# michel-aractingi/soloRL

Hardware: AMD Instinct MI355X
Metric: env-steps/s (whole node) Solo12 walk, 4096 envs/GPU (higher is better)
Workload: dtype f32

## Files before the change

solorl_amd/csrc/solorl_hip.hip:

```cpp
#include <hip/hip_runtime.h>

#include <cmath>
#include <cstddef>
#include <cstdio>
#include <cstdlib>
#include <cstring>
#include <utility>
#include <string>
#include <vector>

#include "../../include/solorl.h"
#include "dynamics.hpp"
#include "perturb.hpp"

using namespace solo;

#ifndef SOLO_TU_PART
#define SOLO_TU_PART -1
#endif
extern "C" __attribute__((visibility("hidden"))) int solorl_fail_(int code, const char* msg);

namespace {

#if SOLO_TU_PART == -1 || SOLO_TU_PART == 4
// ... 444 lines not shown
SD void pol_fma(PolBatch<KB>& B, int K4, int k0, unsigned xoff, unsigned xoff_a, float (&c)[4], float (&a)[4]) {
  asm volatile("" ::: "memory");
#pragma unroll
  for (int kk = 0; kk < KB; kk++) { POL_PIN4(B.c[kk]); POL_PIN4(B.a[kk]); }
#pragma unroll
  for (int kk = 0; kk < KB; kk++)
    if (k0 + kk < K4) {
#pragma unroll
      for (int e = 0; e < 4; e++) {
        const nfloat4 xc = reinterpret_cast<const nfloat4*>(solo_smem + e * POL_ENV_BYTES + xoff)[k0 + kk];
        const nfloat4 xa = xoff_a == xoff ? xc : reinterpret_cast<const nfloat4*>(solo_smem + e * POL_ENV_BYTES + xoff_a)[k0 + kk];
        c[e] = pol_dot4(B.c[kk], xc, c[e]); a[e] = pol_dot4(B.a[kk], xa, a[e]);
      }
    }
}
SD void pol_act_store(const float (&c)[4], const float (&a)[4], unsigned yoff, int lane) {
#pragma unroll
  for (int e = 0; e < 4; e++) {
    float* y = reinterpret_cast<float*>(solo_smem + e * POL_ENV_BYTES + yoff);
    y[lane] = pol_tanh(c[e]); y[64 + lane] = pol_tanh(a[e]);
  }
}

template <int A>
SD void policy_tail_team(const PolicyTail& P, int O, int col, int t, idx_t env, bool valid) {
  float* const buf = reinterpret_cast<float*>(solo_smem + (unsigned)col * POL_ENV_BYTES);
  float* const h2 = buf + 224;
  const int lane = threadIdx.x & 63, O4 = O >> 2;
  static_assert(A < 15, "the critic head sits on lane 15");
  const bool head = t < A || t == 15;
  constexpr unsigned H1 = 96u * 4u, H2 = 224u * 4u;
  float c[4], a[4];
  PolBatch<11> w1a, w1b;
  PolBatch<8> w2a, w2b;
  nfloat4 whb[16];
  pol_load(w1a, P.cw0, P.aw0, O4, 0, lane);
  pol_load(w1b, P.cw0, P.aw0, O4, 11, lane);
#pragma unroll
  for (int e = 0; e < 4; e++) { c[e] = P.cb0[lane]; a[e] = P.ab0[lane]; }
  pol_fma(w1a, O4, 0, 0u, 0u, c, a);
  pol_load(w2a, P.cw1, P.aw1, 16, 0, lane);
  pol_fma(w1b, O4, 11, 0u, 0u, c, a);
  pol_act_store(c, a, H1, lane);
  pol_load(w2b, P.cw1, P.aw1, 16, 8, lane);
#pragma unroll
  for (int e = 0; e < 4; e++) { c[e] = P.cb1[lane]; a[e] = P.ab1[lane]; }
  TEAM_SYNC();
  pol_fma(w2a, 16, 0, H1, H1 + 256u, c, a);
  {
    gfloat4* wh = (gfloat4*)(t == 15 ? P.cw2 : P.mw + (size_t)(head ? t : 0) * 64);
#pragma unroll
    for (int k = 0; k < 16; k++) whb[k] = wh[k];
    asm volatile("" ::: "memory");
  }
  pol_fma(w2b, 16, 8, H1, H1 + 256u, c, a);
  pol_act_store(c, a, H2, lane);
  TEAM_SYNC();
  float out = 0.f;
  {
    asm volatile("" ::: "memory");
#pragma unroll
    for (int k = 0; k < 16; k++) POL_PIN4(whb[k]);
    const nfloat4* x = reinterpret_cast<const nfloat4*>(t == 15 ? h2 : h2 + 64);
    float o0 = t == 15 ? P.cb2[0] : P.mb[head ? t : 0], o1 = 0.f;
#pragma unroll
    for (int k = 0; k < 16; k += 2) { o0 = pol_dot4(whb[k], x[k], o0); o1 = pol_dot4(whb[k + 1], x[k + 1], o1); }
    out = head ? o0 + o1 : 0.f;
  }
  float lp = 0.f, act = out;
  if (t < A) {
    const float ls = P.logstd[t];
    const float nz = P.noise ? P.noise[(size_t)env * A + t] : 0.f;
    act = out + __expf(ls) * nz;
    lp = -0.5f * nz * nz - ls - POL_HALF_LOG_2PI;
  }
  lp = team_sum16(lp);
  if (valid) {
    if (t < A) P.action[(size_t)env * A + t] = act;
    if (t == 15) P.value[env] = out;
    if (t == 0) P.logp[env] = lp;
  }
}

template <typename T, int ROBOT, bool DUO = false>
SD void step_team(T* __restrict__ sf, int* __restrict__ si, const T* __restrict__ snf, const int* __restrict__ sni, int M,
                  const Layout& L, int N, const EnvParams& P, const PhysParams<T>& pp, const float* __restrict__ actions,
                  const Outputs& out, int mode) {
  using RB = Robot<ROBOT>;
  constexpr int NQ = RB::NQ, NPS = 13 + 2 * NQ;
  using LDS = RowLds<T, 4>;
  using CH = typename TeamCtx<T, ROBOT, LDS>::type;
  static_assert(sizeof(PhysState<T, NQ>) == NPS * sizeof(T), "PhysState is the HBM field order pos, quat, v, w, q, qd");
#ifdef SOLO_WAVE_TIMING
  long long wts_[11];
  for (int i_ = 0; i_ < 11; i_++) wts_[i_] = 0;
  const long long wr0_ = wall_clock64();
  if (threadIdx.x < 16) solo::solo_pt_acc[threadIdx.x] = 0;
  __syncthreads();
  wts_[0] = clock64();
#endif
  const unsigned wlane = DUO ? (threadIdx.x & 63u) : threadIdx.x;
  const int t = wlane & 15, col = wlane >> 4;
  const unsigned blk = (blockIdx.x & 7u) * (gridDim.x >> 3) + (blockIdx.x >> 3);
  idx_t e = (idx_t)blk * 4 + col;
  const bool valid = e < (idx_t)N;
  if (!valid) e = (idx_t)N - 1;
  const bool lead = valid && t == 0;
  LDS lds; lds.lanes = 4; lds.lane = col;
  if (P.lds_poison_on) {
    using TC = TeamCtx<T, ROBOT, LDS>;
    unsigned* w = reinterpret_cast<unsigned*>(solo_smem);
    for (unsigned k = wlane; k < TC::bytes / 4; k += 64) w[k] = P.lds_poison;
    __syncthreads();
  }
  const CH ch{col};
  SubCtx<T, ROBOT>& C = ch.get();
  T* const psv = reinterpret_cast<T*>(&C.ps);
  if constexpr (DUO) {
    if (blk * 4u >= (unsigned)N) return;
    if (__builtin_amdgcn_readfirstlane(threadIdx.x >> 6)) {
#pragma unroll 1
      for (int ss = 0; ss < P.frame_skip; ss++)
        substep_team_helper<T, ROBOT>(pp, lds, t, lead, valid, ss + 1 < P.frame_skip);
      duo_join_rows<T, ROBOT>();
      return;
    }
    if (!valid && t == 0) { C.mask = 0; C.nc = 0; C.nlim_total = 0; C.lsel = 0; C.smask = 0; }
  }
  idx_t env = 0;
  T a_t = T(0);
  if (valid) {
    env = P.linear_ids ? e : (idx_t)si[SX(I_ENVID, e, NI)];
    for (int f = t; f < NPS; f += 16) psv[f] = sf[SX(L.pos + f, e, L.NF)];
    if (t < NER) C.erec[t] = sf[SX(L.goal + t, e, L.NF)];
    if (t < 3) C.irec[t] = si[SX(t, e, NI)];
    for (int p = t; p < NPRIM; p += 16) C.lamp[p] = sf[SX(L.lam + p, e, L.NF)];
    if (t < NQ && mode == MODE_STEP) a_t = (T)actions[env * NQ + t];
  }
  static_assert(I_TIMESTEP == IR_TIMESTEP && I_MASK == IR_MASK && I_RNG == IR_RNG, "counter order");
  TEAM_SYNC();
  WT_STAMP(1);
  if (valid && t < NQ) {
    const T c = a_t < T(-1) ? T(-1) : (a_t > T(1) ? T(1) : a_t);
    T tq;
    if (P.control == SOLORL_CONTROL_TORQUE) tq = c * T(P.max_torque);
    else tq = clampv(T(P.kp) * (c * pp.qlim - C.ps.q[t]) - T(P.kd) * C.ps.qd[t], T(P.max_torque));
    C.tau_base[t] = mode == MODE_STEP ? tq : T(0);
    if (out.tau && mode == MODE_STEP) out.tau[env * NQ + t] = (float)tq;
  }
  const T asq = team_sum16(a_t * a_t);
  WT_STAMP(2);
  constexpr int HK = (DMAX + 15) / 16;
  T hk0[HK], hk1[HK];
#pragma unroll
  for (int k = 0; k < HK; k++) { hk0[k] = T(0); hk1[k] = T(0); }
  T csk[HK];
  if (L.H > 0) team_current_state<T, ROBOT, HK>(C, P.task, L.D, t, csk);
  TEAM_SYNC();
  if (lead) {
    C.erec[ER_XYPREV] = C.ps.pos.x; C.erec[ER_XYPREV + 1] = C.ps.pos.y;
    C.tmy = C.erec[ER_TMY];
    if constexpr (DUO) C.R0 = quat_to_mat(C.ps.qx, C.ps.qy, C.ps.qz, C.ps.qw);
  }
  if (valid && L.H > 0) {
#pragma unroll
    for (int k = 0; k < HK; k++) {
      const int d = t + 16 * k;
      if (d < L.D) {
        const T c = csk[k];
        for (int lv = L.H - 1; lv >= 2; lv--)
          sf[SX(L.hist + lv * HSTRIDE + d, e, L.NF)] = sf[SX(L.hist + (lv - 1) * HSTRIDE + d, e, L.NF)];
        if (L.H >= 2) { hk1[k] = sf[SX(L.hist + d, e, L.NF)]; sf[SX(L.hist + HSTRIDE + d, e, L.NF)] = hk1[k]; }
        sf[SX(L.hist + d, e, L.NF)] = c;
        hk0[k] = c;
      } else if (d < ((L.D + 3) & ~3)) {
        sf[SX(L.hist + d, e, L.NF)] = T(0);
        for (int lv = 1; lv < L.H; lv++) sf[SX(L.hist + lv * HSTRIDE + d, e, L.NF)] = T(0);
      }
    }
  }
  WT_STAMP(3);
#pragma unroll 1
  for (int ss = 0; ss < P.frame_skip; ss++) {
    const T sc = (ss == 0 || P.hold_torque) ? T(1) : T(0);
    if (valid && t < NQ) C.tau[t] = C.tau_base[t] * sc;
    const int m = substep_team<T, ROBOT, LDS, DUO>(pp, sf + SX(L.lam, e, L.NF), 4u, lds, t, lead, valid);
    if (lead) C.irec[IR_MASK] = m;
  }
  if constexpr (DUO) {
    duo_join_rows<T, ROBOT>();
  }
  WT_STAMP(4);
// ... 102 lines not shown
    if (with_policy) {
      TEAM_SYNC();
      policy_tail_team<NQ>(out.pol, L.D * (1 + L.H), col, t, env, valid);
    }
  }
  WT_STAMP(9);
#ifdef SOLO_WAVE_TIMING
  __builtin_amdgcn_s_waitcnt(0);
  if (threadIdx.x == 0 && blockIdx.x < solo::SOLO_WT_WAVES) {
    wts_[10] = clock64();
    unsigned long long* w_ = solo::solo_wave_times[blockIdx.x];
    w_[0] = (unsigned long long)(wts_[3] - wts_[0]); w_[1] = (unsigned long long)(wts_[4] - wts_[3]); w_[2] = (unsigned long long)(wts_[10] - wts_[4]);
    w_[3] = (unsigned long long)(wall_clock64() - wr0_);
    for (int i_ = 0; i_ < 10; i_++) w_[6 + i_] = (unsigned long long)(wts_[i_ + 1] > wts_[i_] && wts_[i_] ? wts_[i_ + 1] - wts_[i_] : 0);
    for (int i_ = 0; i_ < 10; i_++) w_[16 + i_] = solo::solo_pt_acc[i_];
    for (int i_ = 10; i_ < 14; i_++) w_[18 + i_] = solo::solo_pt_acc[i_];
  }
#endif
}

template <typename T, int ROBOT>
__global__ void __launch_bounds__(64)
step_kernel(T* __restrict__ sf, int* __restrict__ si, const T* __restrict__ snf, const int* __restrict__ sni, int M,
            Layout L, int N, EnvParams P, PhysParams<T> pp, const float* __restrict__ actions, Outputs out, int mode) {
  step_body<T, ROBOT>(sf, si, snf, sni, M, L, N, P, pp, actions, out, mode);
}

#ifndef SOLO_WAVES_PER_SIMD
#define SOLO_WAVES_PER_SIMD 2
#endif
template <typename T, int ROBOT>
__global__ void __launch_bounds__(64, sizeof(T) == 8 ? 1 : SOLO_WAVES_PER_SIMD)
step_kernel_team(T* __restrict__ sf, int* __restrict__ si, const T* __restrict__ snf, const int* __restrict__ sni, int M,
                 Layout L, int N, EnvParams P, PhysParams<T> pp, const float* __restrict__ actions, Outputs out, int mode) {
  step_team<T, ROBOT>(sf, si, snf, sni, M, L, N, P, pp, actions, out, mode);
}

template <typename T, int ROBOT>
__global__ void __launch_bounds__(128, SOLO_WAVES_PER_SIMD)
duo_kernel_team(T* __restrict__ sf, int* __restrict__ si, const T* __restrict__ snf, const int* __restrict__ sni, int M,
                Layout L, int N, EnvParams P, PhysParams<T> pp, const float* __restrict__ actions, Outputs out, int mode) {
  static_assert(sizeof(T) == 4, "the helper wavefront is an fp32 kernel");
  step_team<T, ROBOT, true>(sf, si, snf, sni, M, L, N, P, pp, actions, out, mode);
}

template <typename T> struct RolloutArgs {
  T* sf; int* si; const T* snf; const int* sni; int M;
  Layout L; int N; EnvParams P; PhysParams<T> pp;
  const float* actions; Outputs out;
  int mode;
  int K, pol_last;
};
template <typename T> SD T* row_adv(T* p, size_t n) { return p ? p + n : p; }
template <typename T, int ROBOT>
__global__ void __launch_bounds__(64, sizeof(T) == 8 ? 1 : SOLO_WAVES_PER_SIMD)
rollout_kernel_team(const RolloutArgs<T> args) {
  using RA = RolloutArgs<T>;
  typedef const __attribute__((address_space(4))) char* kptr;
  constexpr size_t A = Robot<ROBOT>::NQ;
  const int K = args.K;
#pragma unroll 1
  for (int k = 0; k < K; k++) {
    kptr ap = (kptr)__builtin_amdgcn_kernarg_segment_ptr();
    asm volatile("" : "+s"(ap));
    const RA& a = *(const RA*)ap;
    const size_t r = (size_t)k * (size_t)a.N, O = (size_t)(a.L.D * (1 + a.L.H));
    Outputs o = a.out;
    o.obs += r * O; o.rew += r; o.done += r;
    o.timeout = row_adv(o.timeout, r); o.success = row_adv(o.success, r); o.nan_reset = row_adv(o.nan_reset, r);
    o.ep_len = row_adv(o.ep_len, r); o.ep_rew = row_adv(o.ep_rew, r); o.goals = row_adv(o.goals, r);
    o.dr0 = row_adv(o.dr0, r); o.dr1 = row_adv(o.dr1, r); o.dr2 = row_adv(o.dr2, r); o.dr3 = row_adv(o.dr3, r); o.dr4 = row_adv(o.dr4, r);
    o.tau = row_adv(o.tau, r * A);
    if (o.pol.value) {
      if (k + 1 < K || a.pol_last) {
        const size_t r1 = r + (size_t)a.N;
        o.pol.value += r1; o.pol.logp += r1; o.pol.action += r1 * A; o.pol.noise = row_adv(o.pol.noise, r1 * A);
      } else o.pol.value = nullptr;
    }
    step_team<T, ROBOT>(a.sf, a.si, a.snf, a.sni, a.M, a.L, a.N, a.P, a.pp, a.actions + r * A, o, a.mode);
    TEAM_SYNC();
  }
}

template <typename T, int ROBOT, bool MASKED>
__global__ void reset_kernel(T* sf, int* si, const T* snf, const int* sni, int M, Layout L, int N, EnvParams P, float* obs,
                             const unsigned char* mask) {
  const idx_t e = (idx_t)blockIdx.x * blockDim.x + threadIdx.x;
  if (e >= (idx_t)N) return;
  if constexpr (MASKED) { if (!mask[si[SX(I_ENVID, e, NI)]]) return; }
  Env<T, Robot<ROBOT>::NQ> E;
  load_env(E, sf, si, L, (idx_t)N, e);
  const idx_t env = (idx_t)si[SX(I_ENVID, e, NI)];
  reset_from_snapshot<T, ROBOT>(E, sf, L, (idx_t)N, e, env, snf, sni, M, P);
  if (obs) write_obs<T, ROBOT>(E, sf, L, (idx_t)N, e, env, P.task, obs);
  store_env(E, sf, si, L, (idx_t)N, e);
  si[SX(I_NEEDRESET, e, NI)] = 0;
}

template <typename T, int ROBOT>
__global__ void obs_kernel(const T* sf, const int* si, Layout L, int N, int task, float* obs) {
  const idx_t e = (idx_t)blockIdx.x * blockDim.x + threadIdx.x;
  if (e >= (idx_t)N) return;
  Env<T, Robot<ROBOT>::NQ> E;
  load_env(E, sf, si, L, (idx_t)N, e);
  write_obs<T, ROBOT>(E, sf, L, (idx_t)N, e, (idx_t)si[SX(I_ENVID, e, NI)], task, obs);
}

template <typename T>
__global__ void init_pose_kernel(T* sf, int* si, Layout L, int N, T tmy) {
  const idx_t e = (idx_t)blockIdx.x * blockDim.x + threadIdx.x;
  if (e >= (idx_t)N) return;
  for (int f = 0; f < L.NF; f++) sf[SX(f, e, L.NF)] = T(0);
  sf[SX(L.pos + 2, e, L.NF)] = T(0.35);
  sf[SX(L.quat + 3, e, L.NF)] = T(1);
  sf[SX(L.tmy, e, L.NF)] = tmy;
  for (int k = 0; k < NI; k++) si[SX(k, e, NI)] = 0;
  si[SX(I_NEEDRESET, e, NI)] = 1;
  si[SX(I_ENVID, e, NI)] = (int)e;
}

template <typename T>
__global__ void copy_env_kernel(const T* sf, const int* si, int N, int src, T* df, int* di, int M, int dst, int NF) {
  const int f = blockIdx.x * blockDim.x + threadIdx.x;
  if (f < NF) df[SX(f, (idx_t)dst, NF)] = sf[SX(f, (idx_t)src, NF)];
  if (f < NI) di[SX(f, (idx_t)dst, NI)] = si[SX(f, (idx_t)src, NI)];
}

__global__ void __launch_bounds__(256) sort_perm_kernel(const int* __restrict__ si, int N, int* __restrict__ perm) {
  __shared__ int cnt[256][9];
  __shared__ int base[9];
  const int t = threadIdx.x, nt = blockDim.x;
  const int chunk = (N + nt - 1) / nt, lo = t * chunk, hi = lo + chunk < N ? lo + chunk : N;
  int c[9] = {0, 0, 0, 0, 0, 0, 0, 0, 0};
  for (int i = lo; i < hi; i++) { int k = __popc(si[SX(I_MASK, (idx_t)i, NI)] & 0xFFFFFF); k = k > 8 ? 8 : k; c[k]++; }
#pragma unroll
  for (int k = 0; k < 9; k++) cnt[t][k] = c[k];
  __syncthreads();
  if (t < 9) {
    int run = 0;
    for (int j = 0; j < nt; j++) { int v = cnt[j][t]; cnt[j][t] = run; run += v; }
    base[t] = run;
  }
  __syncthreads();
  if (t == 0) { int run = 0; for (int k = 0; k < 9; k++) { int v = base[k]; base[k] = run; run += v; } }
  __syncthreads();
  int off[9];
#pragma unroll
  for (int k = 0; k < 9; k++) off[k] = base[k] + cnt[t][k];
  for (int i = lo; i < hi; i++) {
    int k = __popc(si[SX(I_MASK, (idx_t)i, NI)] & 0xFFFFFF); k = k > 8 ? 8 : k;
    int d = 0;
#pragma unroll
    for (int q = 0; q < 9; q++) if (q == k) d = off[q]++;
    perm[d] = i;
  }
}

template <typename T>
__global__ void gather_state_kernel(const T* __restrict__ sf, const int* __restrict__ si, const int* __restrict__ perm, int N,
                                    int NF, T* __restrict__ df, int* __restrict__ di) {
  const int j = blockIdx.x * blockDim.x + threadIdx.x;
  if (j >= N) return;
  const int src = perm[j];
  const int f = blockIdx.y;
  if (f < NF) df[SX(f, (idx_t)j, NF)] = sf[SX(f, (idx_t)src, NF)];
  else di[SX(f - NF, (idx_t)j, NI)] = si[SX(f - NF, (idx_t)src, NI)];
// ... 155 lines not shown
                const float* __restrict__ vpred, const float* __restrict__ ret, int m, int A, float clip, float value_coef,
                int clipped_value, float* __restrict__ g_mean, float* __restrict__ g_values, float* __restrict__ part) {
  extern __shared__ float red[];
  const int i = blockIdx.x * blockDim.x + threadIdx.x;
  const bool on = i < m;
  const float inv_m = 1.0f / (float)m;
  float vl = 0.f, al = 0.f, glp = 0.f;
  float lp = 0.f;
  if (on) {
    for (int j = 0; j < A; j++) {
      const float ls = logstd[j];
      const float z = (action[(size_t)i * A + j] - mean[(size_t)i * A + j]) * __expf(-ls);
      lp += -0.5f * z * z - ls - 0.91893853320467274178f;
    }
    const float ratio = __expf(lp - old_logp[i]);
    const float a = adv[i];
    const float s1 = ratio * a;
    const float rc = fminf(fmaxf(ratio, 1.0f - clip), 1.0f + clip);
    const float s2 = rc * a;
    al = -fminf(s1, s2);
    const float inside = (ratio >= 1.0f - clip && ratio <= 1.0f + clip) ? 1.0f : 0.0f;
    const float w = s1 < s2 ? 1.0f : (s1 > s2 ? inside : 0.5f * (1.0f + inside));
    glp = -a * ratio * w * inv_m;
    const float v = values[i], r = ret[i];
    const float u = v - r;
    float gv;
    if (clipped_value) {
      const float dvp = v - vpred[i];
      const float vc = vpred[i] + fminf(fmaxf(dvp, -clip), clip);
      const float wv = vc - r;
      const float ins = (dvp >= -clip && dvp <= clip) ? 1.0f : 0.0f;
      const float uu = u * u, ww = wv * wv;
      vl = 0.5f * fmaxf(uu, ww);
      gv = uu > ww ? u : (uu < ww ? wv * ins : 0.5f * (u + wv * ins));
    } else { vl = 0.5f * u * u; gv = u; }
    g_values[i] = value_coef * gv * inv_m;
  }
  auto block_sum = [&](float x) -> float {
    red[threadIdx.x] = x;
    __syncthreads();
    for (int s = 128; s > 0; s >>= 1) { if ((int)threadIdx.x < s) red[threadIdx.x] += red[threadIdx.x + s]; __syncthreads(); }
    const float r = red[0];
    __syncthreads();
    return r;
  };
  float* P = part + (size_t)blockIdx.x * (3 + A);
  const float svl = block_sum(vl), sal = block_sum(al);
  if (threadIdx.x == 0) { P[0] = svl; P[1] = sal; P[2] = (float)(min(m - (int)(blockIdx.x * blockDim.x), (int)blockDim.x)); }
  for (int j = 0; j < A; j++) {
    float gls = 0.f;
    if (on) {
      const float e = __expf(-logstd[j]);
      const float z = (action[(size_t)i * A + j] - mean[(size_t)i * A + j]) * e;
      g_mean[(size_t)i * A + j] = glp * z * e;
      gls = glp * (z * z - 1.0f);
    }
    const float s = block_sum(gls);
    if (threadIdx.x == 0) P[3 + j] = s;
  }
}

}

struct solorl_env {
  solorl_config cfg;
  int N = 0, device = 0, n = 0, D = 0, O = 0, M = 0;
  bool f64 = false, reset_called = false;
  size_t tsize = 4;
  Layout L;
  void* sf = nullptr; int* si = nullptr; void* snf = nullptr; int* sni = nullptr;
  void* sf2 = nullptr; int* si2 = nullptr; int* perm = nullptr;
  bool sort = true;
  uint64_t seed = 0; int64_t id0 = 0;
  double goal_radius = 2.0;
  double* dyn = nullptr;
  std::vector<unsigned> stab_host;
  unsigned* stab = nullptr;
  bool spread = true;
  bool team = false;
  int lds_poison_on = 0; unsigned lds_poison = 0;
  int simds = 1024;
  int pipe_override = -1;
  int helper_override = -1;
  int* pert_countdown = nullptr; unsigned* pert_kicks = nullptr;
  PerturbParams pert{};
};

namespace {

EnvParams make_env_params(const solorl_env* h) {
  EnvParams P;
  const solorl_config& c = h->cfg;
  P.task = c.task; P.control = c.control; P.frame_skip = c.frame_skip; P.episode_length = c.episode_length;
  P.hold_torque = c.hold_torque; P.disable_termination = c.disable_termination;
  P.settle_min = c.settle_min; P.nsettle = c.settle_max - c.settle_min + 1;
  P.seed_lo = (unsigned)h->seed; P.seed_hi = (unsigned)(h->seed >> 32); P.id0 = h->id0;
  P.kp = c.kp; P.kd = c.kd; P.max_torque = c.max_torque; P.reward_dt = c.reward_dt; P.dyn = h->dyn;
  P.lds_poison_on = h->lds_poison_on; P.lds_poison = h->lds_poison;
  P.use_treadmill = c.use_treadmill; P.tm_offset = (float)c.treadmill_offset;
  P.linear_ids = h->sort ? 0 : 1;
  return P;
}

inline int check_lds_base(const void* kernel) {
  hipFuncAttributes a;
  HIP_TRY(hipFuncGetAttributes(&a, kernel));
  if (a.sharedSizeBytes != (size_t)SOLO_LDS_BASE)
    return fail(SOLORL_ERR_HIP, "step kernel's static LDS size differs from SOLO_LDS_BASE: the phase functions' dynamic-LDS base constant does not hold "
                                "(a -DSOLO_WAVE_TIMING build runs team mode only)");
  return 0;
}

inline int team_grid(int N) { return (((N + 3) / 4) + 7) & ~7; }
inline bool team_pipe(const solorl_env* h, int N) { return h->pipe_override >= 0 ? h->pipe_override != 0 : team_grid(N) <= h->simds; }
inline bool helper_wave_allowed(const solorl_env* h) { return h->team && !h->f64 && !h->sort && team_grid(h->N) <= h->simds; }
inline bool helper_wave_rule(const solorl_env* h) { return h->helper_override != 0 && helper_wave_allowed(h); }
inline bool step_n_one_launch(const solorl_env* h) { return h->team && !h->sort; }

template <typename T, int ROBOT>
PhysParams<T> team_launch_shape(const solorl_env* h, int N, dim3& grid, size_t& smem) {
  grid = dim3(team_grid(N));
  using TeamLds = RowLds<T, 4>;
  smem = TeamCtx<T, ROBOT, TeamLds>::bytes;
  static_assert(sizeof(T) == 8 || TeamCtx<T, ROBOT, TeamLds>::bytes <= 20480, "team-mode LDS must allow 8 workgroups per CU (two wavefronts per SIMD)");
  PhysParams<T> pp = make_phys<T>(h->cfg);
  pp.mode = (pp.mode & ~PhysParams<T>::M_PIPE) | (team_pipe(h, N) ? PhysParams<T>::M_PIPE : 0);
  return pp;
}

template <typename T, int ROBOT>
int prepare_kernels(const solorl_env* h) {
  if (int rc = check_lds_base(h->team ? reinterpret_cast<const void*>(step_kernel_team<T, ROBOT>) : reinterpret_cast<const void*>(step_kernel<T, ROBOT>))) return rc;
  if constexpr (sizeof(T) == 4)
    if (helper_wave_rule(h))
      if (int rc = check_lds_base(reinterpret_cast<const void*>(duo_kernel_team<T, ROBOT>))) return rc;
  if (step_n_one_launch(h))
    if (int rc = check_lds_base(reinterpret_cast<const void*>(rollout_kernel_team<T, ROBOT>))) return rc;
  if (!h->team)
    HIP_TRY(hipFuncSetAttribute(reinterpret_cast<const void*>(step_kernel<T, ROBOT>), hipFuncAttributeMaxDynamicSharedMemorySize,
                                (int)RowLds<T>::bytes(sizeof(T) == 8 ? 32 : 64)));
  return 0;
}

template <typename T, int ROBOT>
int launch_step(solorl_env* h, T* sf, int* si, int N, const float* actions, const Outputs& out, int mode, hipStream_t st) {
  if (h->team) {
    dim3 grid;
    size_t team_smem = 0;
    const PhysParams<T> pp = team_launch_shape<T, ROBOT>(h, N, grid, team_smem);
    if constexpr (sizeof(T) == 4) {
      if (helper_wave_rule(h)) {
        hipLaunchKernelGGL((duo_kernel_team<T, ROBOT>), grid, dim3(128), team_smem, st, sf, si, (const T*)h->snf, (const int*)h->sni, h->M, h->L, N,
                           make_env_params(h), pp, actions, out, mode);
        HIP_TRY(hipGetLastError());
        return 0;
      }
    }
    hipLaunchKernelGGL((step_kernel_team<T, ROBOT>), grid, dim3(64), team_smem, st, sf, si, (const T*)h->snf, (const int*)h->sni, h->M, h->L, N,
                       make_env_params(h), pp, actions, out, mode);
    HIP_TRY(hipGetLastError());
    return 0;
  }
  const int EPB = RowLds<T>::LANES;
  size_t smem = RowLds<T>::bytes(EPB);
  if (h->spread && (N + EPB - 1) / EPB <= 256) smem = RowLds<T>::bytes(sizeof(T) == 8 ? 32 : 64);
  dim3 grid((N + EPB - 1) / EPB), block(EPB);
  hipLaunchKernelGGL((step_kernel<T, ROBOT>), grid, block, smem, st, sf, si, (const T*)h->snf, (const int*)h->sni, h->M, h->L, N,
                     make_env_params(h), make_phys<T>(h->cfg), actions, out, mode);
  HIP_TRY(hipGetLastError());
  return 0;
}

template <typename T, int ROBOT>
int launch_rollout(solorl_env* h, T* sf, int* si, int N, const float* actions, const Outputs& out, int K, int pol_last, hipStream_t st) {
  dim3 grid, block(64);
  RolloutArgs<T> a;
  size_t smem = 0;
  a.pp = team_launch_shape<T, ROBOT>(h, N, grid, smem);
  a.sf = sf; a.si = si; a.snf = (const T*)h->snf; a.sni = (const int*)h->sni; a.M = h->M; a.L = h->L; a.N = N; a.P = make_env_params(h);
  a.actions = actions; a.out = out; a.mode = MODE_STEP; a.K = K; a.pol_last = pol_last;
  hipLaunchKernelGGL((rollout_kernel_team<T, ROBOT>), grid, block, smem, st, a);
  HIP_TRY(hipGetLastError());
  return 0;
}

}

#define SOLO_LAUNCH_ARGS solorl_env* h, void* sf, int* si, int N, const float* actions, const void* out, int mode, void* st
#define SOLO_ROLLOUT_ARGS solorl_env* h, void* sf, int* si, int N, const float* actions, const void* out, int K, int pol_last, void* st
#define SOLO_DECLARE_PART(K_) \
  extern "C" __attribute__((visibility("hidden"))) int solorl_prepare_part##K_(const solorl_env* h); \
  extern "C" __attribute__((visibility("hidden"))) int solorl_launch_part##K_(SOLO_LAUNCH_ARGS); \
  extern "C" __attribute__((visibility("hidden"))) int solorl_rollout_part##K_(SOLO_ROLLOUT_ARGS);
SOLO_DECLARE_PART(0) SOLO_DECLARE_PART(1) SOLO_DECLARE_PART(2) SOLO_DECLARE_PART(3)
#define SOLO_DEFINE_PART(K_, T_, R_) \
  extern "C" int solorl_prepare_part##K_(const solorl_env* h) { return prepare_kernels<T_, R_>(h); } \
  extern "C" int solorl_launch_part##K_(SOLO_LAUNCH_ARGS) { \
    return launch_step<T_, R_>(h, (T_*)sf, si, N, actions, *(const Outputs*)out, mode, (hipStream_t)st); } \
  extern "C" int solorl_rollout_part##K_(SOLO_ROLLOUT_ARGS) { \
    return launch_rollout<T_, R_>(h, (T_*)sf, si, N, actions, *(const Outputs*)out, K, pol_last, (hipStream_t)st); }
#if SOLO_TU_PART == -1 || SOLO_TU_PART == 0
SOLO_DEFINE_PART(0, float, 0)
#endif
#if SOLO_TU_PART == -1 || SOLO_TU_PART == 1
SOLO_DEFINE_PART(1, float, 1)
#endif
#if SOLO_TU_PART == -1 || SOLO_TU_PART == 2
SOLO_DEFINE_PART(2, double, 0)
#endif
#if SOLO_TU_PART == -1 || SOLO_TU_PART == 3
SOLO_DEFINE_PART(3, double, 1)
#endif

#if SOLO_TU_PART == -1 || SOLO_TU_PART == 4
namespace {

template <typename F> auto with_type(const solorl_env* h, F&& f) { return h->f64 ? f(double{}) : f(float{}); }
template <typename F> auto with_instantiation(const solorl_env* h, F&& f) {
  return with_type(h, [&](auto t) {
    return h->cfg.robot == SOLORL_ROBOT_SOLO12 ? f(t, std::integral_constant<int, 1>{}) : f(t, std::integral_constant<int, 0>{});
  });
}

int part_index(const solorl_env* h) { return 2 * (h->f64 ? 1 : 0) + (h->cfg.robot == SOLORL_ROBOT_SOLO12 ? 1 : 0); }
constexpr decltype(&solorl_launch_part0) PART_LAUNCH[4] = {solorl_launch_part0, solorl_launch_part1, solorl_launch_part2, solorl_launch_part3};
constexpr decltype(&solorl_rollout_part0) PART_ROLLOUT[4] = {solorl_rollout_part0, solorl_rollout_part1, solorl_rollout_part2, solorl_rollout_part3};
constexpr decltype(&solorl_prepare_part0) PART_PREPARE[4] = {solorl_prepare_part0, solorl_prepare_part1, solorl_prepare_part2, solorl_prepare_part3};

int dispatch_step(solorl_env* h, void* sf, int* si, int N, const float* actions, const Outputs& out, int mode, hipStream_t st) {
  return PART_LAUNCH[part_index(h)](h, sf, si, N, actions, &out, mode, st);
}

int dispatch_rollout(solorl_env* h, const float* actions, const Outputs& out, int K, int pol_last, hipStream_t st) {
  return PART_ROLLOUT[part_index(h)](h, h->sf, h->si, h->N, actions, &out, K, pol_last, st);
}

Outputs make_outputs(float* obs_out, float* reward_out, uint8_t* done_out, const solorl_info_soa* info) {
  Outputs o; memset(&o, 0, sizeof o);
  o.obs = obs_out; o.rew = reward_out; o.done = done_out;
  if (info) {
    o.timeout = info->timeout; o.success = info->success; o.nan_reset = info->nan_reset; o.ep_len = info->episode_length;
    o.ep_rew = info->episode_reward; o.goals = info->goals_reached; o.dr0 = info->dr_stand; o.dr1 = info->dr_joint_pose;
    o.dr2 = info->dr_torque; o.dr3 = info->dr_balance; o.dr4 = info->dr_progress; o.ep_stats = info->ep_stats;
    o.tau = info->applied_torque;
  }
  return o;
}

int check_policy_tail(const solorl_env* h, const solorl_policy_params* p, const char* who) {
  const std::string w(who);
  if (h->f64 || !h->team || h->sort) return fail(SOLORL_ERR_INVALID, w + " needs the fp32 team-mode engine without contact-count sorting (the defaults)");
  if (p->hidden != 64 || p->obs_dim != h->O || p->act_dim != h->n || (h->O & 3) || h->O > 88 || h->L.H > 1)
    return fail(SOLORL_ERR_INVALID, w + ": the policy must be the MLP of hidden size 64 on this env's observation / action sizes, obs_dim a multiple of 4 "
                                        "and at most 88 (zero or one history level)");
  const void* ptrs[] = {p->critic_w0, p->critic_b0, p->critic_w1, p->critic_b1, p->critic_w2, p->critic_b2, p->actor_w0, p->actor_b0, p->actor_w1, p->actor_b1,
                        p->mean_w, p->mean_b, p->logstd};
  for (const void* q : ptrs) if (!q) return fail(SOLORL_ERR_INVALID, w + ": null policy parameter pointer");
  const void* vec[] = {p->critic_w0, p->critic_w1, p->critic_w2, p->actor_w0, p->actor_w1, p->mean_w};
  for (const void* q : vec) if (reinterpret_cast<uintptr_t>(q) & 15u) return fail(SOLORL_ERR_INVALID, w + ": weight matrices must be 16-byte aligned (rows are read as float4)");
  return 0;
}

int step_ready(const solorl_env* h, const float* actions, const float* obs_out, const float* reward_out, const uint8_t* done_out) {
// ... 102 lines not shown
  if (nwaves > solo::SOLO_WT_WAVES) nwaves = solo::SOLO_WT_WAVES;
  if (hipDeviceSynchronize() != hipSuccess) return -3;
  if (out && hipMemcpyFromSymbol(out, HIP_SYMBOL(solo::solo_wave_times), (size_t)nwaves * solo::SOLO_WT_FIELDS * sizeof(unsigned long long)) != hipSuccess) return -3;
  if (reset) {
    void* p = nullptr;
    if (hipGetSymbolAddress(&p, HIP_SYMBOL(solo::solo_wave_times)) != hipSuccess || hipMemset(p, 0, sizeof(solo::solo_wave_times)) != hipSuccess) return -3;
  }
  return 0;
}
#endif

int solorl_compute_returns(const float* rewards, float* value_preds, const float* masks, const float* next_value,
                           float* returns, int T, int N, int use_gae, float gamma, float gae_lambda, int device_id,
                           void* stream) {
  if (!rewards || !value_preds || !masks || !next_value || !returns) return fail(SOLORL_ERR_INVALID, "null array argument");
  if (T < 1 || N < 1) return fail(SOLORL_ERR_INVALID, "T and N must be >= 1");
  int ndev = 0;
  if (hipGetDeviceCount(&ndev) != hipSuccess || ndev < 1) return fail(SOLORL_ERR_NODEVICE, "no HIP device available (no CPU fallback)");
  if (device_id < 0 || device_id >= ndev) return fail(SOLORL_ERR_NODEVICE, "device_id out of range");
  HIP_TRY(hipSetDevice(device_id));
  hipLaunchKernelGGL(returns_kernel, dim3((N + 255) / 256), dim3(256), 0, (hipStream_t)stream, rewards, value_preds, masks,
                     next_value, returns, T, N, use_gae, gamma, gae_lambda);
  HIP_TRY(hipGetLastError());
  return 0;
}
int solorl_ppo_loss(const float* mean, const float* logstd, const float* values, const float* action, const float* old_logp,
                    const float* adv, const float* vpred, const float* ret, int m, int A, float clip, float value_coef,
                    int clipped_value, float* grad_mean, float* grad_values, float* partials, int device_id, void* stream) {
  if (!mean || !logstd || !values || !action || !old_logp || !adv || !vpred || !ret || !grad_mean || !grad_values || !partials)
    return fail(SOLORL_ERR_INVALID, "null array argument");
  if (m < 1 || A < 1) return fail(SOLORL_ERR_INVALID, "m and A must be >= 1");
  int ndev = 0;
  if (hipGetDeviceCount(&ndev) != hipSuccess || ndev < 1) return fail(SOLORL_ERR_NODEVICE, "no HIP device available (no CPU fallback)");
  if (device_id < 0 || device_id >= ndev) return fail(SOLORL_ERR_NODEVICE, "device_id out of range");
  HIP_TRY(hipSetDevice(device_id));
  hipLaunchKernelGGL(ppo_loss_kernel, dim3((m + 255) / 256), dim3(256), 256 * sizeof(float), (hipStream_t)stream, mean, logstd, values,
                     action, old_logp, adv, vpred, ret, m, A, clip, value_coef, clipped_value, grad_mean, grad_values, partials);
  HIP_TRY(hipGetLastError());
  return 0;
}
const char* solorl_version(void) { return "solorl-hip 0.4 (gfx950)"; }
int solorl_abi_version(void) { return SOLORL_ABI_VERSION; }

int solorl_default_config(solorl_config* c, int robot, int task) {
  if (!c) return fail(SOLORL_ERR_INVALID, "null config");
  memset(c, 0, sizeof *c);
  c->robot = robot; c->task = task; c->control = SOLORL_CONTROL_TORQUE;
  c->frame_skip = 4; c->episode_length = 400; c->num_history_stack = 0;
  c->solver_iterations = 50; c->settle_min = 5; c->settle_max = 11; c->precision = SOLORL_PRECISION_F32;
  c->kp = 5.0; c->kd = 0.2; c->max_torque = 3.0; c->sim_dt = 1.0 / 240.0; c->reward_dt = 1.0 / 60.0; c->gravity = 9.81;
  c->erp = 0.2; c->linear_slop = 1e-5; c->warmstart = 0.0; c->damping = 0.04; c->max_velocity = 100.0;
  c->joint_limit = 10.0; c->goal_radius = 2.0;
  c->use_treadmill = 0; c->treadmill_offset = 0.49; c->treadmill_half_width = 0.5; c->treadmill_friction = 0.5;
  c->solver_residual_threshold = 1e-7;
  c->collision_margin = 0.001;
  c->friction_model = SOLORL_FRICTION_CONE; c->contact_erp = 0.08;
  return 0;
}

int solorl_create(const solorl_config* cfg, int num_envs, int device_id, uint64_t seed, int64_t env_id_offset, solorl_env** out) {
  if (!out) return fail(SOLORL_ERR_INVALID, "null out pointer");
  *out = nullptr;
  int rc = check_cfg(cfg);
  if (rc) return rc;
  if (num_envs < 1) return fail(SOLORL_ERR_INVALID, "num_envs must be >= 1");
  int ndev = 0;
  if (hipGetDeviceCount(&ndev) != hipSuccess || ndev < 1) return fail(SOLORL_ERR_NODEVICE, "no HIP device available (the engine has no CPU fallback)");
  if (device_id < 0 || device_id >= ndev) return fail(SOLORL_ERR_NODEVICE, "device_id out of range");
  HIP_TRY(hipSetDevice(device_id));
  solorl_env* h = new solorl_env();
  h->cfg = *cfg; h->N = num_envs; h->device = device_id; h->seed = seed; h->id0 = env_id_offset;
  h->n = cfg->robot == SOLORL_ROBOT_SOLO12 ? 12 : 8;
  h->D = 14 + 2 * h->n + (cfg->task == SOLORL_TASK_POINTGOAL ? 4 : 0);
  h->O = h->D * (1 + cfg->num_history_stack);
  h->f64 = cfg->precision == SOLORL_PRECISION_F64; h->tsize = h->f64 ? 8 : 4;
  h->L = make_layout(h->n, h->D, cfg->num_history_stack);
  h->M = (cfg->settle_max - cfg->settle_min + 1) * (cfg->use_treadmill ? 2 : 1);
  h->goal_radius = cfg->goal_radius;
  {
    if (const char* ev = getenv("SOLORL_SPREAD")) h->spread = atoi(ev) != 0;
    h->team = true;
    if (const char* ev = getenv("SOLORL_TEAM")) h->team = atoi(ev) != 0;
    if (const char* ev = getenv("SOLORL_PGS_PIPE")) h->pipe_override = atoi(ev) != 0;
    if (const char* ev = getenv("SOLORL_HELPER_WAVE")) h->helper_override = atoi(ev) != 0;
    { hipDeviceProp_t prop; if (hipGetDeviceProperties(&prop, device_id) == hipSuccess && prop.multiProcessorCount > 0) h->simds = 4 * prop.multiProcessorCount; }
    if (const char* ev = getenv("SOLORL_POISON_LDS")) { h->lds_poison_on = 1; h->lds_poison = (unsigned)strtoul(ev, nullptr, 0); }
  }
  auto cleanup = [&](int code) { solorl_destroy(h); return code; };
  const size_t Np = ((size_t)num_envs + 3) & ~(size_t)3, Mp = ((size_t)h->M + 3) & ~(size_t)3;
  if ((unsigned long long)h->L.NF * (unsigned long long)Np >= (1ull << 31) ||
      (unsigned long long)(h->L.D * (1 + h->L.H)) * (unsigned long long)num_envs >= (1ull << 31))
    return cleanup(fail(SOLORL_ERR_INVALID, "num_envs too large for 32-bit element indices"));
  if (hipMalloc(&h->sf, h->tsize * h->L.NF * Np) != hipSuccess) return cleanup(fail(SOLORL_ERR_HIP, "hipMalloc state"));
  if (hipMalloc(&h->si, sizeof(int) * NI * Np) != hipSuccess) return cleanup(fail(SOLORL_ERR_HIP, "hipMalloc istate"));
  if (hipMalloc(&h->snf, h->tsize * h->L.NF * Mp) != hipSuccess) return cleanup(fail(SOLORL_ERR_HIP, "hipMalloc snapshot"));
  if (hipMalloc(&h->sni, sizeof(int) * NI * Mp) != hipSuccess) return cleanup(fail(SOLORL_ERR_HIP, "hipMalloc isnapshot"));
  {
    double dyn0[NDYN] = {h->goal_radius, 0.0, 0.0, 0.0};
    if (hipMalloc(&h->dyn, sizeof dyn0) != hipSuccess) return cleanup(fail(SOLORL_ERR_HIP, "hipMalloc dyn"));
    if (hipMemcpy(h->dyn, dyn0, sizeof dyn0, hipMemcpyHostToDevice) != hipSuccess) return cleanup(fail(SOLORL_ERR_HIP, "hipMemcpy dyn"));
  }
  {
    if (h->L.NF > ST_MAXNF) return cleanup(fail(SOLORL_ERR_INVALID, "state layout wider than the batched state kernels' staging block"));
    std::vector<unsigned>& tab = h->stab_host;
    build_state_table(h->L, h->n, tab);
    if (hipMalloc(&h->stab, sizeof(unsigned) * tab.size()) != hipSuccess) return cleanup(fail(SOLORL_ERR_HIP, "hipMalloc state table"));
    if (hipMemcpy(h->stab, tab.data(), sizeof(unsigned) * tab.size(), hipMemcpyHostToDevice) != hipSuccess) return cleanup(fail(SOLORL_ERR_HIP, "hipMemcpy state table"));
  }
  h->sort = false;
  if (const char* ev = getenv("SOLORL_SORT")) h->sort = atoi(ev) != 0 && num_envs >= 2;
  if (h->helper_override == 1 && !helper_wave_allowed(h))
    return cleanup(fail(SOLORL_ERR_INVALID, "SOLORL_HELPER_WAVE=1 needs the fp32 team-mode engine without contact-count sorting and a batch of at most "
                                            "one workgroup (four envs) per SIMD of the device: " + std::to_string(4 * h->simds) + " envs here"));
  if (h->sort) {
    if (hipMalloc(&h->sf2, h->tsize * h->L.NF * Np) != hipSuccess) return cleanup(fail(SOLORL_ERR_HIP, "hipMalloc state2"));
    if (hipMalloc(&h->si2, sizeof(int) * NI * Np) != hipSuccess) return cleanup(fail(SOLORL_ERR_HIP, "hipMalloc istate2"));
    if (hipMalloc(&h->perm, sizeof(int) * (size_t)num_envs) != hipSuccess) return cleanup(fail(SOLORL_ERR_HIP, "hipMalloc perm"));
  }
  if ((rc = PART_PREPARE[part_index(h)](h))) return cleanup(rc);
  rc = with_type(h, [&](auto t) {
    using T = decltype(t);
    hipLaunchKernelGGL(init_pose_kernel<T>, dim3((num_envs + 255) / 256), dim3(256), 0, 0, (T*)h->sf, h->si, h->L, num_envs, T(0));
    return build_snapshots_t<T>(h);
  });
  if (rc) return cleanup(rc);
  if (hipDeviceSynchronize() != hipSuccess) return cleanup(fail(SOLORL_ERR_HIP, "device sync after create"));
  *out = h;
  return 0;
}

int solorl_destroy(solorl_env* h) {
  if (!h) return 0;
  hipSetDevice(h->device);
  if (h->sf) hipFree(h->sf);
  if (h->si) hipFree(h->si);
  if (h->snf) hipFree(h->snf);
  if (h->sni) hipFree(h->sni);
  if (h->sf2) hipFree(h->sf2);
  if (h->si2) hipFree(h->si2);
  if (h->perm) hipFree(h->perm);
  if (h->dyn) hipFree(h->dyn);
  if (h->stab) hipFree(h->stab);
  if (h->pert_countdown) hipFree(h->pert_countdown);
  if (h->pert_kicks) hipFree(h->pert_kicks);
  delete h;
  return 0;
}

int solorl_dims(const solorl_env* h, int* obs_dim, int* act_dim, int* num_envs) {
  if (!h) return fail(SOLORL_ERR_INVALID, "null handle");
  if (obs_dim) *obs_dim = h->O;
  if (act_dim) *act_dim = h->n;
  if (num_envs) *num_envs = h->N;
  return 0;
}

int solorl_get_property(const solorl_env* h, const char* name, double* value) {
  if (!h || !name || !value) return fail(SOLORL_ERR_INVALID, "null argument");
  const std::string n(name);
  if (n == "lanes_per_env") *value = h->team ? 16 : 1;
  else if (n == "sweep_variant") {
    if (h->cfg.solver_residual_threshold > 0) *value = 2;
    else if (!h->team) *value = 1;
    else *value = team_pipe(h, h->N) ? 1 : 0;
  } else if (n == "max_contacts") *value = MAX_CONTACTS;
  else if (n == "max_limit_rows") *value = MAX_LIMITS;
  else if (n == "f64") *value = h->f64 ? 1 : 0;
  else if (n == "sort") *value = h->sort ? 1 : 0;
  else if (n == "step_n_one_launch") *value = step_n_one_launch(h) ? 1 : 0;
  else if (n == "helper_wave") *value = helper_wave_rule(h) ? 1 : 0;
  else return fail(SOLORL_ERR_INVALID, "unknown property: " + n);
  return 0;
}

int solorl_reset(solorl_env* h, float* obs_out, void* stream) {
  if (!h) return fail(SOLORL_ERR_INVALID, "null handle");
  if (int rc = launch_reset<false>(h, nullptr, obs_out, stream)) return rc;
  h->reset_called = true;
  return 0;
}

int solorl_step(solorl_env* h, const float* actions, float* obs_out, float* reward_out, uint8_t* done_out,
                const solorl_info_soa* info, void* stream) {
  if (!h) return fail(SOLORL_ERR_INVALID, "null handle");
  if (int rc = step_ready(h, actions, obs_out, reward_out, done_out)) return rc;
  Outputs o = make_outputs(obs_out, reward_out, done_out, info);
  if (h->sort) {
    hipStream_t st = (hipStream_t)stream;
    hipLaunchKernelGGL(sort_perm_kernel, dim3(1), dim3(256), 0, st, (const int*)h->si, h->N, h->perm);
    with_type(h, [&](auto t) {
      using T = decltype(t);
      hipLaunchKernelGGL(gather_state_kernel<T>, dim3((h->N + 255) / 256, h->L.NF + NI), dim3(256), 0, st, (const T*)h->sf, (const int*)h->si,
                         (const int*)h->perm, h->N, h->L.NF, (T*)h->sf2, h->si2);
    });
    HIP_TRY(hipGetLastError());
    std::swap(h->sf, h->sf2); std::swap(h->si, h->si2);
  }
  return dispatch_step(h, h->sf, h->si, h->N, actions, o, MODE_STEP, (hipStream_t)stream);
}

int solorl_step_act(solorl_env* h, const float* actions, float* obs_out, float* reward_out, uint8_t* done_out, const solorl_info_soa* info,
                    const solorl_policy_params* p, const float* noise, float* value_out, float* action_out, float* logp_out, void* stream) {
  if (!h) return fail(SOLORL_ERR_INVALID, "null handle");
  if (!p || !value_out || !action_out || !logp_out) return fail(SOLORL_ERR_INVALID, "solorl_step_act: null policy argument");
  if (int rc = check_policy_tail(h, p, "solorl_step_act")) return rc;
  if (int rc = step_ready(h, actions, obs_out, reward_out, done_out)) return rc;
  Outputs o = make_outputs(obs_out, reward_out, done_out, info);
  o.pol = make_policy_tail(p, noise, value_out, action_out, logp_out);
  return dispatch_step(h, h->sf, h->si, h->N, actions, o, MODE_STEP, (hipStream_t)stream);
}

static solorl_info_soa info_row(const solorl_info_soa& in, size_t r, size_t A) {
  solorl_info_soa o = in;
  auto adv = [r](auto* p) { return p ? p + r : p; };
  o.timeout = adv(in.timeout); o.success = adv(in.success); o.nan_reset = adv(in.nan_reset); o.episode_length = adv(in.episode_length);
  o.episode_reward = adv(in.episode_reward); o.goals_reached = adv(in.goals_reached); o.dr_stand = adv(in.dr_stand);
  o.dr_joint_pose = adv(in.dr_joint_pose); o.dr_torque = adv(in.dr_torque); o.dr_balance = adv(in.dr_balance); o.dr_progress = adv(in.dr_progress);
  o.applied_torque = in.applied_torque ? in.applied_torque + r * A : nullptr;
  return o;
}

int solorl_step_n(solorl_env* h, int K, const float* actions, float* obs_out, float* reward_out, uint8_t* done_out, const solorl_info_soa* info,
                  void* stream) {
  if (K < 1) return fail(SOLORL_ERR_INVALID, "solorl_step_n: K must be >= 1");
  if (!h) return fail(SOLORL_ERR_INVALID, "null handle");
  if (int rc = step_ready(h, actions, obs_out, reward_out, done_out)) return rc;
  if (!step_n_one_launch(h)) {
    const size_t N = (size_t)h->N, O = (size_t)h->O, A = (size_t)h->n;
    for (int k = 0; k < K; k++) {
      const size_t r = (size_t)k * N;
      solorl_info_soa ik;
      if (info) ik = info_row(*info, r, A);
      if (int rc = solorl_step(h, actions + r * A, obs_out + r * O, reward_out + r, done_out + r, info ? &ik : nullptr, stream)) return rc;
    }
    return 0;
  }
  if (K == 1) return dispatch_step(h, h->sf, h->si, h->N, actions, make_outputs(obs_out, reward_out, done_out, info), MODE_STEP, (hipStream_t)stream);
  return dispatch_rollout(h, actions, make_outputs(obs_out, reward_out, done_out, info), K, 0, (hipStream_t)stream);
}

int solorl_rollout(solorl_env* h, int K, float* actions, float* obs_out, float* reward_out, uint8_t* done_out, const solorl_info_soa* info,
                   const solorl_policy_params* p, const float* noise, float* value_out, float* logp_out, int policy_after_last, void* stream) {
  if (K < 1) return fail(SOLORL_ERR_INVALID, "solorl_rollout: K must be >= 1");
  if (!h) return fail(SOLORL_ERR_INVALID, "null handle");
  if (!p || !value_out || !logp_out) return fail(SOLORL_ERR_INVALID, "solorl_rollout: null policy argument");
  if (int rc = check_policy_tail(h, p, "solorl_rollout")) return rc;
  if (int rc = step_ready(h, actions, obs_out, reward_out, done_out)) return rc;
  Outputs o = make_outputs(obs_out, reward_out, done_out, info);
  o.pol = make_policy_tail(p, noise, value_out, actions, logp_out);
  if (K == 1) {
    if (policy_after_last) { o.pol.value = value_out + h->N; o.pol.logp = logp_out + h->N; o.pol.action = actions + (size_t)h->N * h->n; if (noise) o.pol.noise = noise + (size_t)h->N * h->n; }
    else o.pol = PolicyTail{};
    return dispatch_step(h, h->sf, h->si, h->N, actions, o, MODE_STEP, (hipStream_t)stream);
// ... 191 lines not shown
```

solorl_amd/ppo/graphs.py:

```python
import os

import torch
import torch.nn as nn

from . import dist as D
from .fused import ClipAdam, MiniBatchGrad, fused_ppo_loss, policy_act, policy_kernels_supported, policy_params
from .ppo import PPO


def _kernels_enabled():
    return os.environ.get("SOLORL_PPO_KERNELS", "1") != "0"


def capture_kwargs():
    return {"capture_error_mode": "thread_local"} if D.world() > 1 else {}


def _side_stream_warmup(fn, iters=3):
    s = torch.cuda.Stream()
    s.wait_stream(torch.cuda.current_stream())
    with torch.cuda.stream(s):
        for _ in range(iters):
            fn()
    torch.cuda.current_stream().wait_stream(s)


def probe_captured_allreduce(dev, numel, replays=8, time_it=False):
    import time
    import torch.distributed as dist
    w, r = D.world(), D.rank()

    def agree(flag):
        t = torch.tensor([1 if flag else 0], device=dev)
        dist.all_reduce(t, op=dist.ReduceOp.MIN)
        return bool(t.item())

    probe = torch.zeros(int(numel), device=dev)
    dist.all_reduce(probe)
    torch.cuda.synchronize()
    g, captured = None, True
    try:
        g = torch.cuda.CUDAGraph()
        with torch.cuda.graph(g, **capture_kwargs()):
            dist.all_reduce(probe, op=dist.ReduceOp.SUM)
    except Exception:
        captured = False
    if not agree(captured):
        return False, None
    ok = True
    for k in range(1, replays + 1):
        probe.fill_(float(k * (r + 1)))
        g.replay()
        torch.cuda.synchronize()
        ok = ok and bool((probe == float(k * w * (w + 1) // 2)).all().item())
    ok = agree(ok)
    sec = None
    if ok and time_it:
        probe.zero_()
        torch.cuda.synchronize(); dist.barrier()
        t0 = time.perf_counter()
        for _ in range(50):
            g.replay()
        torch.cuda.synchronize()
        sec = (time.perf_counter() - t0) / 50
    return ok, sec


class GraphedRollout:

    def __init__(self, envs, actor_critic, storage, num_steps, chunk=None):
        self.envs, self.ac, self.storage, self.T = envs, actor_critic, storage, num_steps
        self.chunk = int(os.environ.get("SOLORL_ROLLOUT_CHUNK", "0")) if chunk is None else int(chunk)
        self.windows = None
        self.graph = None

    def _body(self):
        st = self.storage
        assert st.step == 0, "graphed rollouts start at storage step 0"
        fused = _kernels_enabled() and policy_kernels_supported(self.ac)
        if fused:
            self._pp = policy_params(self.ac)
        noise = torch.randn_like(st.actions) if fused else None
        done = torch.empty(self.T, st.num_agents, dtype=torch.uint8, device=st.device)
        self.step_act = bool(fused and os.environ.get("SOLORL_STEP_ACT", "1") != "0" and hasattr(self.envs, "step_act_supported")
                             and self.envs.step_act_supported(self._pp))
        if fused and self.chunk > 0 and hasattr(self.envs, "rollout_supported") and self.envs.rollout_supported(self._pp):
            policy_act(self._pp, st.obs[0], noise[0], st.value_preds[0], st.actions[0], st.action_log_probs[0])
            self.windows = []
            for t0 in range(0, self.T, self.chunk):
                K = min(self.chunk, self.T - t0)
                pal = 1 if t0 + K < self.T else 0
                R = K + pal
                self.envs.rollout_inplace(st.actions[t0:t0 + R], self._pp, noise[t0:t0 + R], st.value_preds[t0:t0 + R], st.action_log_probs[t0:t0 + R],
                                          obs_out=st.obs[t0 + 1:t0 + 1 + K], rew_out=st.rewards[t0:t0 + K], done_out=done[t0:t0 + K], policy_after_last=pal)
                self.windows.append(K)
            torch.sub(torch.ones((), device=st.device), done, out=st.masks[1:].view(self.T, st.num_agents))
            return
        for t in range(self.T):
            if self.step_act:
                if t == 0:
                    policy_act(self._pp, st.obs[0], noise[0], st.value_preds[0], st.actions[0], st.action_log_probs[0])
                if t + 1 < self.T:
                    self.envs.step_act_inplace(st.actions[t], self._pp, noise[t + 1], st.value_preds[t + 1], st.actions[t + 1], st.action_log_probs[t + 1],
                                               obs_out=st.obs[t + 1], rew_out=st.rewards[t], done_out=done[t])
                else:
                    self.envs.step_inplace(st.actions[t], obs_out=st.obs[t + 1], rew_out=st.rewards[t], done_out=done[t])
                continue
            if fused:
                policy_act(self._pp, st.obs[t], noise[t], st.value_preds[t], st.actions[t], st.action_log_probs[t])
            else:
                self.ac.act_into(st.obs[t], st.value_preds[t], st.actions[t], st.action_log_probs[t])
            self.envs.step_inplace(st.actions[t], obs_out=st.obs[t + 1], rew_out=st.rewards[t], done_out=done[t])
        torch.sub(torch.ones((), device=st.device), done, out=st.masks[1:].view(self.T, st.num_agents))

    def _capturable(self):
        sort = hasattr(self.envs, "get_property") and self.envs.get_property("sort") != 0
        return not sort or self.T % 2 == 0

    def __call__(self):
        if not self._capturable():
            from .train import rollout
            return rollout(self.envs, self.ac, self.storage, self.T)
        if self.graph is None:
            g = torch.cuda.CUDAGraph()
            with torch.cuda.graph(g, **capture_kwargs()):
                self._body()
            self.graph = g
        self.graph.replay()


class GraphedPPO(PPO):

    def __init__(self, actor_critic, clip_param, ppo_epoch, mini_batch_size, value_loss_coef, entropy_coef, lr=None,
                 l2_coef=0.0, max_grad_norm=None, use_clipped_value_loss=True, fused_loss=True, fused_mlp=True):
        super().__init__(actor_critic, clip_param, ppo_epoch, mini_batch_size, value_loss_coef, entropy_coef, lr=lr,
                         l2_coef=l2_coef, max_grad_norm=max_grad_norm, use_clipped_value_loss=use_clipped_value_loss)
        self.fused_loss = fused_loss
        self.fused_mlp = fused_mlp and _kernels_enabled() and policy_kernels_supported(actor_critic)
        dev = next(actor_critic.parameters()).device
        self.optimizer = torch.optim.Adam(actor_critic.parameters(), lr=torch.tensor(float(lr), device=dev),
                                          weight_decay=l2_coef, capturable=True, fused=True)
        self._built_for = None

    def _build(self, storage):
        dev = storage.device
        n, m = storage.num_samples, self.mini_batch_size
        flat = lambda x: x.reshape(n, *x.shape[2:])
        self._src = (flat(storage.obs[:-1]), flat(storage.actions), flat(storage.value_preds[:-1]), flat(storage.returns[:-1]),
                     flat(storage.action_log_probs))
        assert all(s.data_ptr() == b.data_ptr() for s, b in zip(self._src, (storage.obs, storage.actions, storage.value_preds,
                                                                            storage.returns, storage.action_log_probs)))
        self._adv = torch.zeros(n, 1, device=dev)
        self._perm = torch.zeros(n, dtype=torch.long, device=dev)
        self._off = torch.zeros((), dtype=torch.long, device=dev)
        self._ar = torch.arange(m, device=dev)
# ... 127 lines not shown
```

Baseline: 29.19 million.

## Add helper-wave multi-step rollout kernel and enable chunked rollout windows by default

Adds a duo_window_team kernel that runs K env steps in one launch using the two-wavefront (helper wave) team layout, where the second wave runs substep helper work. It is used in place of rollout_kernel_team when the helper-wave rule allows, and an optional empty spacer launch (K=0) precedes it. The Python rollout default chunk now equals num_steps, so the windowed single-launch rollout path is active by default. The aim is to combine the helper-wave parallelism with fewer kernel launches per rollout. The cost is an extra launch, 128-thread blocks with a different occupancy, and a new code path.

```diff
diff --git a/solorl_amd/csrc/solorl_hip.hip b/solorl_amd/csrc/solorl_hip.hip
--- a/solorl_amd/csrc/solorl_hip.hip
+++ b/solorl_amd/csrc/solorl_hip.hip
@@ -550,7 +550,7 @@
   }
 }
 
-template <typename T, int ROBOT, bool DUO = false>
+template <typename T, int ROBOT, bool DUO = false, bool WINDOW = false>
 SD void step_team(T* __restrict__ sf, int* __restrict__ si, const T* __restrict__ snf, const int* __restrict__ sni, int M,
                   const Layout& L, int N, const EnvParams& P, const PhysParams<T>& pp, const float* __restrict__ actions,
                   const Outputs& out, int mode) {
@@ -575,7 +575,7 @@
   if (!valid) e = (idx_t)N - 1;
   const bool lead = valid && t == 0;
   LDS lds; lds.lanes = 4; lds.lane = col;
-  if (P.lds_poison_on) {
+  if (!WINDOW && P.lds_poison_on) {
     using TC = TeamCtx<T, ROBOT, LDS>;
     unsigned* w = reinterpret_cast<unsigned*>(solo_smem);
     for (unsigned k = wlane; k < TC::bytes / 4; k += 64) w[k] = P.lds_poison;
@@ -844,6 +844,43 @@
   }
 }
 
+template <typename T, int ROBOT>
+__global__ void __launch_bounds__(128, SOLO_WAVES_PER_SIMD)
+duo_window_team(const RolloutArgs<T> args) {
+  static_assert(sizeof(T) == 4, "the helper wavefront is an fp32 kernel");
+  using RA = RolloutArgs<T>;
+  typedef const __attribute__((address_space(4))) char* kptr;
+  constexpr size_t A = Robot<ROBOT>::NQ;
+  if (args.P.lds_poison_on) {
+    using TC = TeamCtx<T, ROBOT, RowLds<T, 4>>;
+    unsigned* w = reinterpret_cast<unsigned*>(solo_smem);
+    for (unsigned k = threadIdx.x & 63u; k < TC::bytes / 4; k += 64) w[k] = args.P.lds_poison;
+    __syncthreads();
+  }
+  const int K = args.K;
+#pragma unroll 1
+  for (int k = 0; k < K; k++) {
+    kptr ap = (kptr)__builtin_amdgcn_kernarg_segment_ptr();
+    asm volatile("" : "+s"(ap));
+    const RA& a = *(const RA*)ap;
+    const size_t r = (size_t)k * (size_t)a.N, O = (size_t)(a.L.D * (1 + a.L.H));
+    Outputs o = a.out;
+    o.obs += r * O; o.rew += r; o.done += r;
+    o.timeout = row_adv(o.timeout, r); o.success = row_adv(o.success, r); o.nan_reset = row_adv(o.nan_reset, r);
+    o.ep_len = row_adv(o.ep_len, r); o.ep_rew = row_adv(o.ep_rew, r); o.goals = row_adv(o.goals, r);
+    o.dr0 = row_adv(o.dr0, r); o.dr1 = row_adv(o.dr1, r); o.dr2 = row_adv(o.dr2, r); o.dr3 = row_adv(o.dr3, r); o.dr4 = row_adv(o.dr4, r);
+    o.tau = row_adv(o.tau, r * A);
+    if (o.pol.value) {
+      if (k + 1 < K || a.pol_last) {
+        const size_t r1 = r + (size_t)a.N;
+        o.pol.value += r1; o.pol.logp += r1; o.pol.action += r1 * A; o.pol.noise = row_adv(o.pol.noise, r1 * A);
+      } else o.pol.value = nullptr;
+    }
+    step_team<T, ROBOT, true, true>(a.sf, a.si, a.snf, a.sni, a.M, a.L, a.N, a.P, a.pp, a.actions + r * A, o, a.mode);
+    TEAM_SYNC();
+  }
+}
+
 template <typename T, int ROBOT, bool MASKED>
 __global__ void reset_kernel(T* sf, int* si, const T* snf, const int* sni, int M, Layout L, int N, EnvParams P, float* obs,
                              const unsigned char* mask) {
@@ -1165,6 +1202,7 @@
   int simds = 1024;
   int pipe_override = -1;
   int helper_override = -1;
+  int window_spacer = 1;
   int* pert_countdown = nullptr; unsigned* pert_kicks = nullptr;
   PerturbParams pert{};
 };
@@ -1199,6 +1237,7 @@
 inline bool helper_wave_allowed(const solorl_env* h) { return h->team && !h->f64 && !h->sort && team_grid(h->N) <= h->simds; }
 inline bool helper_wave_rule(const solorl_env* h) { return h->helper_override != 0 && helper_wave_allowed(h); }
 inline bool step_n_one_launch(const solorl_env* h) { return h->team && !h->sort; }
+inline bool window_helper_rule(const solorl_env* h) { return step_n_one_launch(h) && helper_wave_rule(h); }
 
 template <typename T, int ROBOT>
 PhysParams<T> team_launch_shape(const solorl_env* h, int N, dim3& grid, size_t& smem) {
@@ -1217,8 +1256,12 @@
   if constexpr (sizeof(T) == 4)
     if (helper_wave_rule(h))
       if (int rc = check_lds_base(reinterpret_cast<const void*>(duo_kernel_team<T, ROBOT>))) return rc;
-  if (step_n_one_launch(h))
+  if (step_n_one_launch(h)) {
+    if constexpr (sizeof(T) == 4)
+      if (window_helper_rule(h))
+        if (int rc = check_lds_base(reinterpret_cast<const void*>(duo_window_team<T, ROBOT>))) return rc;
     if (int rc = check_lds_base(reinterpret_cast<const void*>(rollout_kernel_team<T, ROBOT>))) return rc;
+  }
   if (!h->team)
     HIP_TRY(hipFuncSetAttribute(reinterpret_cast<const void*>(step_kernel<T, ROBOT>), hipFuncAttributeMaxDynamicSharedMemorySize,
                                 (int)RowLds<T>::bytes(sizeof(T) == 8 ? 32 : 64)));
@@ -1262,6 +1305,19 @@
   a.pp = team_launch_shape<T, ROBOT>(h, N, grid, smem);
   a.sf = sf; a.si = si; a.snf = (const T*)h->snf; a.sni = (const int*)h->sni; a.M = h->M; a.L = h->L; a.N = N; a.P = make_env_params(h);
   a.actions = actions; a.out = out; a.mode = MODE_STEP; a.K = K; a.pol_last = pol_last;
+  if constexpr (sizeof(T) == 4) {
+    if (window_helper_rule(h)) {
+      if (h->window_spacer) {
+        RolloutArgs<T> s = a;
+        s.K = 0;
+        hipLaunchKernelGGL((duo_window_team<T, ROBOT>), grid, dim3(128), smem, st, s);
+        HIP_TRY(hipGetLastError());
+      }
+      hipLaunchKernelGGL((duo_window_team<T, ROBOT>), grid, dim3(128), smem, st, a);
+      HIP_TRY(hipGetLastError());
+      return 0;
+    }
+  }
   hipLaunchKernelGGL((rollout_kernel_team<T, ROBOT>), grid, block, smem, st, a);
   HIP_TRY(hipGetLastError());
   return 0;
@@ -1530,6 +1586,7 @@
     h->team = true;
     if (const char* ev = getenv("SOLORL_TEAM")) h->team = atoi(ev) != 0;
     if (const char* ev = getenv("SOLORL_PGS_PIPE")) h->pipe_override = atoi(ev) != 0;
+    if (const char* ev = getenv("SOLORL_WINDOW_SPACER")) h->window_spacer = atoi(ev) != 0;
     if (const char* ev = getenv("SOLORL_HELPER_WAVE")) h->helper_override = atoi(ev) != 0;
     { hipDeviceProp_t prop; if (hipGetDeviceProperties(&prop, device_id) == hipSuccess && prop.multiProcessorCount > 0) h->simds = 4 * prop.multiProcessorCount; }
     if (const char* ev = getenv("SOLORL_POISON_LDS")) { h->lds_poison_on = 1; h->lds_poison = (unsigned)strtoul(ev, nullptr, 0); }
@@ -1617,6 +1674,7 @@
   else if (n == "sort") *value = h->sort ? 1 : 0;
   else if (n == "step_n_one_launch") *value = step_n_one_launch(h) ? 1 : 0;
   else if (n == "helper_wave") *value = helper_wave_rule(h) ? 1 : 0;
+  else if (n == "window_helper_wave") *value = window_helper_rule(h) ? 1 : 0;
   else return fail(SOLORL_ERR_INVALID, "unknown property: " + n);
   return 0;
 }
diff --git a/solorl_amd/ppo/graphs.py b/solorl_amd/ppo/graphs.py
--- a/solorl_amd/ppo/graphs.py
+++ b/solorl_amd/ppo/graphs.py
@@ -70,7 +70,7 @@
 
     def __init__(self, envs, actor_critic, storage, num_steps, chunk=None):
         self.envs, self.ac, self.storage, self.T = envs, actor_critic, storage, num_steps
-        self.chunk = int(os.environ.get("SOLORL_ROLLOUT_CHUNK", "0")) if chunk is None else int(chunk)
+        self.chunk = int(os.environ.get("SOLORL_ROLLOUT_CHUNK", num_steps)) if chunk is None else int(chunk)
         self.windows = None
         self.graph = None
 
```

New measurement: 29.24 million, median of 6. About the same (+0.2%).
